# rounak-meyur/revs-admm

Hardware: NVIDIA B200
Metric: home_hours_scheduled_per_sec (higher is better)
Workload: dtype f64

## Files before the change

revs-admm_b200/csrc/kernels.cuh:

```cuda
#pragma once
#include <vector>

#include "common.cuh"

namespace revs {

struct HomeParams {
    const double* load;
    const double* p_est;
    const double* p_sch;
    const int* iter;
    const double* gamma;
    const double* cost;
    const uint8_t* has_ev;
    const double* rating;
    const int* start;
    const int* end;
    const int* n_min;
    const int* n_max;
    double* p_sch_new;
    double* p_ev;
    double* dsum;
    int first;
    int* infeasible;
// ... 47 lines not shown
    ResidualOut* res;
    PeerReduce peer;
    double* partials;
    int Hp, T;
    double kappa, tol, count;
};

cudaError_t launch_dual_update(const DualParams& P, cudaStream_t stream);

struct QpParams {
    const FeederDev* feeders;
    const double* Rpool;
    const double* rn2;
    const double* rmax;
    int* cand;
    int* queue;
    const double* z_t;
    double* lam_t;
    double* g_t;
    double* v_t;
    void* gbf_t;
    const float* v32_t;
    int* wcount;
    int* widx;
    int* status;
    int* inner_ok;
    int* n_running;
    unsigned long long* newton_its;
    int* max_ws;
    unsigned long long* flops;
    unsigned long long* cols;
    int* n_failed;
    int* cls;
    int* n_cls;
    const int* order;
    const int* order_count;
    int4* order4;
    int sweep;
    int list0, nlists;
    int list_extra;
    int warp_m_max;
    int warp_m_max_big;
    int ncols;
    long long* trace;
    unsigned long long* dbg;
    int T;
    int64_t Hp;
    double u, tol;
    int init;
    int inner_max;
    int* round_ctr;
    unsigned long long cond_round;
    int use_cond;
};

struct RoundEndParams {
    const int* n_running;
    const int* n_failed;
    const int* infeasible;
    int* round_ctr;
    int* noconv;
    unsigned long long* rounds_total;
    int round_max;
    unsigned long long cond_round;
    int use_cond;
};
cudaError_t launch_round_end(const RoundEndParams& P, cudaStream_t stream);

struct ClassGateParams {
    const int* order_count;
    unsigned long long cond[kQpClasses];
    int first_gated;
};
cudaError_t launch_class_gate(const ClassGateParams& P, cudaStream_t stream);
cudaError_t qp_warp_prepare();
cudaError_t screen_prepare();
cudaError_t screen_tc5_prepare();

cudaError_t launch_utility_qp(const QpParams& P, int grid, int cls, cudaStream_t stream);
int qp_warp_max_n();
cudaError_t launch_qp_init(const QpParams& P, int max_warp_n, cudaStream_t stream);
int qp_warp_ctas_per_sm();
int qp_warp_m_max_default();
cudaError_t launch_utility_qp_warp(const QpParams& P, int nj, int ctas_per_sm, cudaStream_t stream);
cudaError_t launch_utility_qp_fast(const QpParams& P, cudaStream_t stream);
cudaError_t launch_order_columns(const QpParams& P, int mode, int* order, int* order_count, cudaStream_t stream);

struct NewtonZone {
    int feeder;
    int nn, nlev, n;
    int wn;
    int col0;
    int64_t node_off;
    int64_t home_off;
    int64_t lvl_off;
    int64_t ws_off;
    double scale;
};
struct NewtonParams {
    const NewtonZone* zones;
    int n_zones;
    const int* lvl;
    const int* parent;
    const int2* child;
    const int2* homes;
    const double* rho;
    const int* hlist;
    const int* hnode;
    double* ws;
    double4* ws4;
    double2* ws2;
    int* wsi;
    int64_t ws_stride;
    const FeederDev* feeders;
    const double* z_t;
    double* lam_t;
    double* g_t;
    int* status;
    int* inner_ok;
    int* wcount;
    int* noconv;
    double* dbg_dump;
    int dbg_dump_col, dbg_dump_outer, dbg_dump_guess;
    double* dbg_trace;
    int* dbg_col;
    unsigned long long* newton_its;
    unsigned long long* cols;
    unsigned long long* flops;
    int* max_ws;
    int T;
    int64_t Hp;
    double u, tol;
};
struct NewtonZoneHost {
    std::vector<int> lvl, parent, child0, nchild, home0, nhome, hlist, hnode;
    std::vector<double> rho;
    double scale = 1.0;
};
void newton_build_zone(int n_nodes, const int* parent, const double* r, int n_res, const int* res_node, NewtonZoneHost& Z);
cudaError_t launch_tree_newton(const NewtonParams& P, int n_cols, cudaStream_t stream);
constexpr int kNewtonWsDoubles = 18, kNewtonWs4 = 3, kNewtonWs2 = 2, kNewtonWsInts = 3;

int contract_tile_rows(int T);
cudaError_t launch_contract(const ContractProblem* d_problems, const ContractTile* d_tiles, int n_tiles,
                            int T, int mode, double v2, cudaStream_t stream);

cudaError_t launch_gather_wait(const unsigned long long* flags, int world, unsigned long long seq, int* timeout, cudaStream_t s);

int screen_tile_rows();
cudaError_t launch_to_bf16(const double* in, void* out, size_t n, cudaStream_t s);
cudaError_t launch_screen(const ScreenProblem* d_problems, const ContractTile* d_tiles, int n_tiles, int T, double thr,
                          cudaStream_t stream);

int screen_tc5_tile_rows();
size_t screen_tc5_map_bytes();
uint32_t screen_tc5_box_rows_a();
uint32_t screen_tc5_box_rows_b();
cudaError_t screen_tc5_encode(void* host_map, const void* gptr, uint64_t rows, uint64_t cols, uint64_t pitch_elems,
                              uint32_t box_rows);
cudaError_t launch_screen_tc5(const ScreenProblem* d_problems, const ContractTile* d_tiles, int n_tiles, const void* d_maps_a,
                              const void* d_map_b, const int* d_b_col0, int T, double thr, cudaStream_t stream);

cudaError_t launch_sens_voltage(const int* parent, const double* cumr, const int* row_node,
                                const int* res_node, int n_rows, int n_res, double* out, int ld,
                                cudaStream_t s);
cudaError_t launch_sens_voltage_batched(const FeederDev* feeders, int n_feeders, int max_n, const int64_t* node_off,
// ... 171 lines not shown
```

revs-admm_b200/csrc/revs_capi.cu:

```cuda
#include <chrono>
#include <cstdarg>
#include <cstdio>
#include <cstring>
#include <algorithm>
#include <cstdlib>
#include <cmath>
#include <mutex>
#include <string>
#include <vector>

#include "../../include/revs_admm.h"
#include "kernels.cuh"

using namespace revs;

namespace {

thread_local std::string g_err;

int fail(int code, const char* fmt, ...) {
    char buf[512];
    va_list ap;
    va_start(ap, fmt);
    vsnprintf(buf, sizeof buf, fmt, ap);
// ... 962 lines not shown
    const size_t HT = (size_t)hp * T;

#define TRY(x)                                                                                     \
    do {                                                                                           \
        cudaError_t e_ = (x);                                                                      \
        if (e_ != cudaSuccess) {                                                                   \
            free_all(s);                                                                           \
            delete s;                                                                              \
            return fail(REVS_ERR_CUDA, "%s failed: %s", #x, cudaGetErrorString(e_));               \
        }                                                                                          \
    } while (0)
    int prio_lo = 0, prio_hi = 0;
    TRY(cudaDeviceGetStreamPriorityRange(&prio_lo, &prio_hi));
    s->prio_lo = prio_lo;
    s->prio_hi = prio_hi;
    TRY(cudaStreamCreateWithPriority(&s->sU, cudaStreamNonBlocking, prio_hi));
    TRY(cudaStreamCreateWithPriority(&s->sH, cudaStreamNonBlocking, prio_lo));
    TRY(cudaEventCreateWithFlags(&s->evV, cudaEventDisableTiming));
    for (int cl = 0; cl < kQpClasses; ++cl) {
        TRY(cudaStreamCreateWithPriority(&s->sQ[cl], cudaStreamNonBlocking, prio_hi));
        TRY(cudaEventCreateWithFlags(&s->evQ[cl], cudaEventDisableTiming));
    }
    TRY(cudaEventCreateWithFlags(&s->evHomeDone, cudaEventDisableTiming));
    TRY(cudaEventCreateWithFlags(&s->evDualDone, cudaEventDisableTiming));
    TRY(cudaEventCreate(&s->evT0));
    TRY(cudaEventCreate(&s->evT1));
    TRY(dalloc(&s->d_feeders, (size_t)n_feeders));
    TRY(cudaMemcpy(s->d_feeders, s->feeders.data(), sizeof(FeederDev) * n_feeders, cudaMemcpyHostToDevice));
    TRY(dalloc(&s->d_Rpool, (size_t)rp));
    TRY(dalloc(&s->d_rn2, (size_t)hp));
    TRY(dalloc(&s->d_rmax, (size_t)hp));
    TRY(dalloc(&s->d_cand, (size_t)s->ncols));
    TRY(dalloc(&s->d_stage, (size_t)s->H * (T + 1)));
    {
        std::vector<int64_t> hmap((size_t)s->H);
        for (int f = 0; f < n_feeders; ++f)
            for (int64_t i = feeder_off[f]; i < feeder_off[f + 1]; ++i) hmap[i] = s->feeders[f].off + (i - feeder_off[f]);
        TRY(dalloc(&s->d_hmap, hmap.size()));
        TRY(cudaMemcpy(s->d_hmap, hmap.data(), hmap.size() * sizeof(int64_t), cudaMemcpyHostToDevice));
    }
    s->Rpool_elems = (size_t)rp;
    TRY(cudaMalloc(&s->d_Rbf, (size_t)(rp ? rp : 1) * 2));
    TRY(cudaMemset(s->d_Rbf, 0, (size_t)(rp ? rp : 1) * 2));
    TRY(cudaMalloc(&s->d_gbf, HT * 2));
    TRY(cudaMemset(s->d_gbf, 0, HT * 2));
    TRY(dalloc(&s->d_v32, HT));
    if (getenv("REVS_EXACT_GEMM")) s->screen = false;
    TRY(dalloc(&s->d_load, HT));
    TRY(dalloc(&s->d_pest, HT));
    TRY(dalloc(&s->d_psch[0], HT));
    TRY(dalloc(&s->d_psch[1], HT));
    TRY(dalloc(&s->d_gamma, HT));
    TRY(dalloc(&s->d_pev, HT));
    TRY(dalloc(&s->d_soc, (size_t)hp * (T + 1)));
    TRY(dalloc(&s->d_has_ev, (size_t)hp));
    TRY(dalloc(&s->d_rating, (size_t)hp));
    TRY(dalloc(&s->d_capacity, (size_t)hp));
    TRY(dalloc(&s->d_initial, (size_t)hp));
    TRY(dalloc(&s->d_indconst, (size_t)hp));
    TRY(dalloc(&s->d_start, (size_t)hp));
    TRY(dalloc(&s->d_end, (size_t)hp));
    TRY(dalloc(&s->d_nmin, (size_t)hp));
    TRY(dalloc(&s->d_nmax, (size_t)hp));
    TRY(dalloc(&s->d_zero_i, (size_t)hp));
    TRY(dalloc(&s->d_cost, (size_t)T));
    TRY(dalloc(&s->d_zt, HT));
    TRY(dalloc(&s->d_lamt, HT));
    TRY(dalloc(&s->d_gt, HT));
    TRY(dalloc(&s->d_vt, HT));
    TRY(dalloc(&s->d_wcount, (size_t)s->ncols));
    TRY(dalloc(&s->d_widx, (size_t)s->ncols * kWMax));
    TRY(dalloc(&s->d_status, (size_t)s->ncols));
    TRY(dalloc(&s->d_innerok, (size_t)s->ncols));
    TRY(dalloc(&s->d_cls, (size_t)s->ncols));
    TRY(dalloc(&s->d_order, (size_t)s->ncols * kQpClasses));
    TRY(dalloc(&s->d_order4, (size_t)s->ncols * (kQpLists - kQpClasses)));
    if (hp >= (int64_t)1 << 31 || (rp >> 4) >= (int64_t)1 << 31) s->use_warp_kernel = false;
    TRY(dalloc(&s->d_order_count, (size_t)2 * kQpLists));
    TRY(dalloc(&s->d_cnt, (size_t)1));
    TRY(dalloc(&s->d_respart, (size_t)2 * ((hp + 31) / 32)));
    TRY(dalloc(&s->d_dsum, (size_t)hp));
    {
        const char* e;
        s->warp_m_max = (e = getenv("REVS_WARP_M_MAX")) ? atoi(e) : qp_warp_m_max_default();
        s->warp_m_max_big = (e = getenv("REVS_WARP_M_MAX_BIG")) ? atoi(e) : s->warp_m_max;
        s->use_fast = !((e = getenv("REVS_NO_FAST")) && atoi(e));
        s->debug = getenv("REVS_DEBUG") != nullptr;
        s->debug_host = getenv("REVS_DEBUG_HOST") != nullptr;
        if ((e = getenv("REVS_NO_GRAPH")) && atoi(e)) s->use_graph = false;
        if ((e = getenv("REVS_DEBUG_TRACE")) && sscanf(e, "%d,%d", &s->trace_iter, &s->trace_round) == 2) s->use_graph = false;
        if ((e = getenv("REVS_DEBUG_TRACE_FILE"))) s->trace_file = e;
        if (s->debug) s->use_graph = false;
    }
    TRY(cudaHostAlloc((void**)&s->h_cnt, sizeof(Counters), cudaHostAllocDefault));
    memset(s->h_cnt, 0, sizeof(Counters));

    {
        int rc2 = build_tables(s);
        if (rc2) { free_all(s); delete s; return rc2; }
    }
#undef TRY
    *out = s;
    return REVS_OK;
}

int revs_destroy(revs_solver* s) {
    if (!s) return REVS_OK;
    free_all(s);
    delete s;
    return REVS_OK;
}

int revs_set_sensitivity(revs_solver* s, int feeder, const double* R_res) {
    if (!s || !R_res || feeder < 0 || feeder >= s->nf) return fail(REVS_ERR_ARG, "bad arguments");
    CU(cudaSetDevice(s->device));
    const FeederDev& fd = s->feeders[feeder];
    if (s->roff_alloc[feeder] < 0)
        return fail(REVS_ERR_ARG, "feeder %d has %d residences (> %d): it runs on its tree, give it with "
                    "revs_set_feeder_tree(s) instead of a dense block", feeder, fd.n, kDenseMaxN);
    if (s->is_newton[feeder]) {
        int rc = set_newton(s, feeder, false);
        if (rc) return rc;
        s->nt_host[feeder] = NewtonZoneHost();
        if ((rc = build_tables(s)) || (rc = rebuild_newton(s))) return rc;
    }
    for (int64_t i = 0; i < (int64_t)fd.n * fd.n; ++i)
        if (!(R_res[i] >= 0.0)) return fail(REVS_ERR_ARG, "sensitivity block of feeder %d has a negative or NaN entry", feeder);
    if (fd.n)
        CU(cudaMemcpy2D(s->d_Rpool + fd.roff, (size_t)fd.np * sizeof(double), R_res, (size_t)fd.n * sizeof(double),
                        (size_t)fd.n * sizeof(double), fd.n, cudaMemcpyHostToDevice));
    s->sens_set[feeder] = 1;
    s->rn2_valid = false;
    return REVS_OK;
}

int revs_set_feeder_tree(revs_solver* s, int feeder, int n_nodes, const int32_t* parent, const double* r,
                         const int32_t* res_node) {
    if (!s || !parent || !r || !res_node || feeder < 0 || feeder >= s->nf || n_nodes <= 0)
        return fail(REVS_ERR_ARG, "bad arguments");
    CU(cudaSetDevice(s->device));
    const FeederDev& fd = s->feeders[feeder];
    std::vector<double> cumr(n_nodes);
    for (int i = 0; i < n_nodes; ++i) {
        if (parent[i] >= i || parent[i] < -1) return fail(REVS_ERR_ARG, "nodes must be topologically ordered (parent[i] < i)");
        if (!(r[i] >= 0.0)) return fail(REVS_ERR_ARG, "negative or NaN resistance at node %d", i);
        cumr[i] = (parent[i] < 0 ? 0.0 : cumr[parent[i]]) + r[i];
    }
    for (int j = 0; j < fd.n; ++j)
        if (res_node[j] < 0 || res_node[j] >= n_nodes) return fail(REVS_ERR_ARG, "res_node[%d] out of range", j);
    Tree& t = s->trees[feeder];
    if (t.d_parent && !t.pooled) { cudaFree(t.d_parent); cudaFree(t.d_cumr); cudaFree(t.d_res_node); }
    t = Tree();
    s->net.valid = false;
    s->net.central_valid = false;
    t.n_nodes = n_nodes;
    CU(dalloc(&t.d_parent, (size_t)n_nodes));
    CU(dalloc(&t.d_cumr, (size_t)n_nodes));
    CU(dalloc(&t.d_res_node, (size_t)fd.np));
    CU(cudaMemcpy(t.d_parent, parent, sizeof(int) * n_nodes, cudaMemcpyHostToDevice));
    CU(cudaMemcpy(t.d_cumr, cumr.data(), sizeof(double) * n_nodes, cudaMemcpyHostToDevice));
    CU(cudaMemcpy(t.d_res_node, res_node, sizeof(int) * fd.n, cudaMemcpyHostToDevice));
    {
        const bool want = fd.n > s->newton_min_n || s->roff_alloc[feeder] < 0;
        if (want != (bool)s->is_newton[feeder]) {
            int rc = set_newton(s, feeder, want);
            if (rc || (rc = build_tables(s))) return rc;
        }
    }
// ... 1454 lines not shown
```

revs-admm_b200/csrc/utility_qp_warp.cu:

```cuda
#include <cstdlib>

#include <cuda_bf16.h>

#include "kernels.cuh"

namespace revs {

namespace {

#ifndef REVS_WARPS_PER_CTA
#define REVS_WARPS_PER_CTA 4
#endif
constexpr int kWarpsPerCta = REVS_WARPS_PER_CTA;
constexpr int kCtasPerSm = 16 / kWarpsPerCta;
constexpr int kHW = kWW + 1;
constexpr int kCacheDoubles = 1024;
constexpr double kArcMinW = 9.5367431640625e-07;
constexpr int kPdasMaxW = 40;
constexpr double kHessShiftW = 1e-12;
constexpr int kAddMaxW = 8;
constexpr int kPassMaxW = 10;
constexpr int kRecheckMaxW = 256;
constexpr int kHysteresisW = 8;

template <int CACHE>
struct WarpSmemT {
    double H[kWW * kHW];
    double L[kWW * kHW];
    double rows[CACHE];
};
#ifndef REVS_WARP_CTAS_SMALL
#define REVS_WARP_CTAS_SMALL (8 / REVS_WARPS_PER_CTA)
#endif
#ifndef REVS_WARP_CTAS_BIG
#define REVS_WARP_CTAS_BIG (8 / REVS_WARPS_PER_CTA)
#endif
#ifndef REVS_WARP_CACHE_BIG
#define REVS_WARP_CACHE_BIG 2560
#endif
template <int NJ> struct WarpCfg {
    static constexpr int kCache = NJ <= 4 ? kCacheDoubles : REVS_WARP_CACHE_BIG;
    static constexpr int kCtas = NJ <= 8 ? (NJ <= 4 ? kCtasPerSm : REVS_WARP_CTAS_SMALL) : REVS_WARP_CTAS_BIG;
};

struct WarpStats {
    unsigned long long its = 0;
    double flops = 0.0;
    int handed = 0, deferred = 0, max_ws = 0, cols = 0;
};

__device__ __forceinline__ double warp_bcast(double v, int src) { return __shfl_sync(0xffffffffu, v, src); }

template <int NJ>
__device__ __forceinline__ void recheck_rows(unsigned candk, const double* __restrict__ R, int ld, int n,
                                             const double (&gj)[NJ], double (&vub)[NJ]) {
    const int lane = threadIdx.x & 31;
    const unsigned full = 0xffffffffu;
    if (!__any_sync(full, candk != 0u)) return;
#pragma unroll 1
    for (int k = 0; k < NJ; ++k) {
        unsigned cand = __ballot_sync(full, (candk >> k) & 1u);
        while (cand) {
            int s[4], cnt = 0;
#pragma unroll
            for (int q = 0; q < 4; ++q) {
                if (cand) { s[q] = __ffs(cand) - 1; cand &= cand - 1; ++cnt; }
                else s[q] = s[0];
            }
            double a[4] = {0.0, 0.0, 0.0, 0.0};
#pragma unroll
            for (int kk = 0; kk < NJ; ++kk) {
                const int jj = lane + 32 * kk;
                if (jj < n) {
#pragma unroll
                    for (int q = 0; q < 4; ++q) a[q] = fma(R[(size_t)(s[q] + 32 * k) * ld + jj], gj[kk], a[q]);
                }
            }
#pragma unroll
            for (int o = 16; o > 0; o >>= 1) {
#pragma unroll
                for (int q = 0; q < 4; ++q) a[q] += __shfl_xor_sync(full, a[q], o);
            }
            double mine = 0.0;
            bool hit = false;
#pragma unroll
            for (int q = 0; q < 4; ++q)
                if (q < cnt && lane == s[q]) { mine = a[q]; hit = true; }
            if (hit) {
#pragma unroll
                for (int kk = 0; kk < NJ; ++kk)
                    if (kk == k) vub[kk] = mine;
            }
        }
    }
}

template <int NJ>
__device__ __forceinline__ void solve_column(const QpParams& P, const int4 ent, WarpSmemT<WarpCfg<NJ>::kCache>& sm, WarpStats& st) {
    constexpr int kCacheD = WarpCfg<NJ>::kCache;
    const int lane = threadIdx.x & 31;
    const unsigned full = 0xffffffffu;
    const int c = ent.x;
    const int n = ent.z & 0xffff, ld = ent.z >> 16;
    const int t = c % P.T;
    const size_t hoff = (size_t)ent.y;
    const double* __restrict__ R = P.Rpool + ((size_t)ent.w << 4);
    const size_t col = (size_t)t * P.Hp + hoff;
    const double* z = P.z_t + col;
    double* lam_g = P.lam_t + col;
    double* g = P.g_t + col;
    const double u = P.u, tol = P.tol;
    int* widx = P.widx + (size_t)c * kWMax;
    const int m_old = P.wcount[c];
    const bool solved_before = P.inner_ok[c] == 1;
    const int wi = lane < kWW ? widx[lane] : 0;

    long long tr_start = 0;
    if (P.trace) asm volatile("mov.u64 %0, %%globaltimer;" : "=l"(tr_start));
    const long long tr_clk0 = clock64();
    const double thr = (1.0 - kScreenMargin) * u;

    double zj[NJ], gj[NJ], g0[NJ], vub[NJ];
    unsigned inw = 0;
    unsigned candk = 0;
    if (P.v32_t) {
        const float* v32 = P.v32_t + col;
        float vf[NJ];
#pragma unroll
        for (int k = 0; k < NJ; ++k) {
            const int jc = min(lane + 32 * k, n - 1);
            zj[k] = z[jc];
            gj[k] = g[jc];
            vf[k] = v32[jc];
        }
        if (lane < (n + 15) / 16) asm volatile("prefetch.global.L2 [%0];" ::"l"(P.rmax + hoff + 16 * lane));
#pragma unroll
        for (int k = 0; k < NJ; ++k) {
            const bool in = lane + 32 * k < n;
            if (!in) { zj[k] = 0.0; gj[k] = 0.0; }
            g0[k] = gj[k];
            const double a = in ? (double)vf[k] : 0.0;
            vub[k] = kScreenUp * a;
            if (in && a > thr) candk |= 1u << k;
        }
    } else {
        const double* v64 = P.v_t + col;
#pragma unroll
        for (int k = 0; k < NJ; ++k) {
            const int jc = min(lane + 32 * k, n - 1);
            zj[k] = z[jc];
            gj[k] = g[jc];
            vub[k] = v64[jc];
        }
#pragma unroll
        for (int k = 0; k < NJ; ++k) {
            if (lane + 32 * k >= n) { zj[k] = 0.0; gj[k] = 0.0; vub[k] = 0.0; }
            g0[k] = gj[k];
        }
    }

    int idx = 0, m = 0;
    double lam = 0.0;
    if (m_old > 0) {
        const double l = lane < m_old ? lam_g[wi] : 0.0;
        const unsigned keep = __ballot_sync(full, lane < m_old && l > 0.0);
        m = __popc(keep);
        const int src = __fns(keep, 0, lane + 1);
        const int si = __shfl_sync(full, wi, src & 31);
        const double sl = __shfl_sync(full, l, src & 31);
        if (lane < m) { idx = si; lam = sl; }
#pragma unroll 1
        for (int a = 0; a < m; ++a) {
            const int h = __shfl_sync(full, idx, a);
            if ((h & 31) == lane) inw |= 1u << (h >> 5);
        }
        candk &= ~inw;
    }

    double flops = 0.0;
    int its_total = 0;
    bool changed = false;
    long long tph[4] = {0, 0, 0, 0}, tq0 = clock64(), tq1;
    int npass = 0;
#define WPHASE(i) do { if (P.trace) { tq1 = clock64(); tph[i] += tq1 - tq0; tq0 = tq1; } } while (0)
    auto trace_out = [&](int kind) {
        if (P.trace && lane == 0) {
            long long tr_end; unsigned smid;
            asm volatile("mov.u64 %0, %%globaltimer;" : "=l"(tr_end));
            asm volatile("mov.u32 %0, %%smid;" : "=r"(smid));
            long long* rec = P.trace + 12 * (size_t)c;
            rec[0] = tr_start; rec[1] = tr_end; rec[2] = smid; rec[3] = ((long long)m << 20) | its_total;
            for (int i = 0; i < 4; ++i) rec[4 + i] = tph[i];
            rec[8] = npass; rec[9] = kind; rec[10] = m_old; rec[11] = clock64() - tr_clk0;
        }
    };
    tph[0] = tq0 - tr_clk0;
    int exit_kind = 0, reason = 0;
    double grad = 0.0;

    for (int pass = 0;; ++pass) {
        recheck_rows<NJ>(candk, R, ld, n, gj, vub);
        candk = 0;
        WPHASE(pass == 0 ? 0 : 3);

        if (pass > 0) {
            const bool row = lane < m;
            unsigned drop = __ballot_sync(full, row && !(lam > 0.0));
            if (drop) {
                const unsigned keep = __ballot_sync(full, row && lam > 0.0);
                while (drop) {
                    const int a = __ffs(drop) - 1;
                    drop &= drop - 1;
                    const int h = __shfl_sync(full, idx, a);
                    const double vr = u - warp_bcast(grad, a);
                    if ((h & 31) == lane) {
#pragma unroll
                        for (int k = 0; k < NJ; ++k)
                            if (k == (h >> 5)) { vub[k] = vr; inw &= ~(1u << k); }
                    }
                }
                m = __popc(keep);
                const int src = __fns(keep, 0, lane + 1);
                const int si = __shfl_sync(full, idx, src & 31);
                const double sl = __shfl_sync(full, lam, src & 31);
                idx = lane < m ? si : 0;
                lam = lane < m ? sl : 0.0;
            }
        }

        int added = 0;
        bool left = false;
        const int room = min(kAddMaxW, kWW - m);
#pragma unroll 1
        for (int r = 0; r <= room; ++r) {
            double best = -1.0;
            int bj = 0x7fffffff;
#pragma unroll
            for (int k = 0; k < NJ; ++k) {
                const int j = lane + 32 * k;
                const double viol = vub[k] - u;
                if (j < n && !((inw >> k) & 1u) && viol > tol && viol > best) { best = viol; bj = j; }
            }
            if (!__any_sync(full, best >= 0.0)) break;
#pragma unroll
            for (int o = 16; o > 0; o >>= 1) {
                const double ob = __shfl_xor_sync(full, best, o);
                const int oj = __shfl_xor_sync(full, bj, o);
                if (ob > best || (ob == best && oj < bj)) { best = ob; bj = oj; }
            }
            if (r == room) { left = true; break; }
            if (lane == m + added) { idx = bj; lam = 0.0; }
            if ((bj & 31) == lane) inw |= 1u << (bj >> 5);
            ++added;
        }
        if (added == 0 && !left) {
            if (pass > 0 || m == 0 || solved_before) break;
        }
        if ((left && m + added == kWW) || pass >= kPassMaxW) { exit_kind = 2; reason = pass >= kPassMaxW ? 2 : 1; break; }
        m += added;
        ++npass;
        const bool row = lane < m;

        const int ncache = min(m, kCacheD / ld);
        __syncwarp();
        {
            const int nchunk = (n + 1) >> 1;
#pragma unroll 1
            for (int a = 0; a < ncache; ++a) {
                const double* src = R + (size_t)__shfl_sync(full, idx, a) * ld;
                const unsigned dst = (unsigned)__cvta_generic_to_shared(sm.rows + a * ld);
                for (int ch = lane; ch < nchunk; ch += 32)
                    asm volatile("cp.async.cg.shared.global [%0], [%1], 16;" ::"r"(dst + 16u * ch), "l"(src + 2 * ch) : "memory");
            }
            asm volatile("cp.async.commit_group;" ::: "memory");
            asm volatile("cp.async.wait_group 0;" ::: "memory");
        }
        __syncwarp();
        auto rowp = [&](int a) -> const double* {
            const int ia = __shfl_sync(full, idx, a);
            return a < ncache ? sm.rows + a * ld : R + (size_t)ia * ld;
        };

        int ok = 0, its = 0;
        bool bail = false;
        WPHASE(1);

        if (m == 1) {
            const double* rp = rowp(0);
            double r1[NJ];
#pragma unroll
            for (int k = 0; k < NJ; ++k) {
                const int j = lane + 32 * k;
                r1[k] = j < n ? rp[j] : 0.0;
            }
            const double l_in = warp_bcast(lam, 0);
            double l = l_in;
#pragma unroll 1
            for (int it = 0; it < 48; ++it) {
                double v = 0.0, S = 0.0;
#pragma unroll
                for (int k = 0; k < NJ; ++k) {
                    const double gk = fmax(zj[k] - r1[k] * l, 0.0);
                    gj[k] = gk;
                    v = fma(r1[k], gk, v);
                    if (gk > 0.0) S = fma(r1[k], r1[k], S);
                }
#pragma unroll
                for (int o = 16; o > 0; o >>= 1) {
                    v += __shfl_xor_sync(full, v, o);
                    S += __shfl_xor_sync(full, S, o);
                }
                ++its;
                const double fr = v - u;
                if ((l > 0.0 ? fabs(fr) : fmax(fr, 0.0)) < tol) { ok = 1; grad = -fr; break; }
                double ln = S > 0.0 ? l + fr / S : 0.0;
                if (ln < 0.0) ln = 0.0;
                if (ln == l) break;
                l = ln;
            }
            flops += 4.0 * n * its;
            lam = lane == 0 ? l : 0.0;
            if (l != l_in) changed = true;
            if (ok && l == l_in) its = 0;
            if (!ok) its = 0;
        }

        if (!ok) {
            const double scale = warp_sum(row ? P.rn2[hoff + idx] : 0.0) / (double)max(m, 1);
            const double shift = kHessShiftW * scale + 1e-300;
            double phi;
            {
                double acc = 0.0;
#pragma unroll
                for (int k = 0; k < NJ; ++k) acc = fma(gj[k], gj[k], acc);
                phi = 0.5 * warp_sum(acc) + u * warp_sum(row ? lam : 0.0);
            }
            double hrow[kWW];
#pragma unroll
            for (int q = 0; q < kWW; ++q) hrow[q] = 0.0;
            unsigned fbits = 0;
            bool have_H = false;
// ... 19 lines not shown
                if (kkt < tol) { ok = 1; break; }

                {
                    int nupd = 0;
                    unsigned nowmask = 0;
#pragma unroll
                    for (int k = 0; k < NJ; ++k)
                        if (gj[k] > 0.0) nowmask |= 1u << k;
                    if (!have_H) {
#pragma unroll 1
                        for (int p = 0; p < m; ++p) {
                            const double* rp_ptr = rowp(p);
                            double rp[NJ];
#pragma unroll
                            for (int k = 0; k < NJ; ++k) {
                                const int j = lane + 32 * k;
                                rp[k] = (j < n && gj[k] > 0.0) ? rp_ptr[j] : 0.0;
                            }
#pragma unroll 1
                            for (int q = 0; q <= p; q += 2) {
                                const double* r0 = rowp(q);
                                const double* r1 = rowp(min(q + 1, p));
                                double a0 = 0.0, a1 = 0.0;
#pragma unroll
                                for (int k = 0; k < NJ; ++k) {
                                    const int j = lane + 32 * k;
                                    if (j < n) { a0 = fma(rp[k], r0[j], a0); a1 = fma(rp[k], r1[j], a1); }
                                }
#pragma unroll
                                for (int o = 16; o > 0; o >>= 1) {
                                    a0 += __shfl_xor_sync(full, a0, o);
                                    a1 += __shfl_xor_sync(full, a1, o);
                                }
                                if (lane == p) {
#pragma unroll
                                    for (int qq = 0; qq < kWW; ++qq) {
                                        if (qq == q) hrow[qq] = a0;
                                        if (qq == q + 1 && q + 1 <= p) hrow[qq] = a1;
                                    }
                                }
                            }
                        }
                        nupd = __reduce_add_sync(full, __popc(nowmask));
                    } else {
#pragma unroll 1
                        for (int k = 0; k < NJ; ++k) {
                            const bool now = (nowmask >> k) & 1u;
                            const bool was = (fbits >> k) & 1u;
                            unsigned chg = __ballot_sync(full, now != was);
                            const unsigned nowb = __ballot_sync(full, now);
                            while (chg) {
                                const int src = __ffs(chg) - 1;
                                chg &= chg - 1;
                                const int j = src + 32 * k;
                                const double sgn = ((nowb >> src) & 1u) ? 1.0 : -1.0;
                                const double ra = row ? (lane < ncache ? sm.rows[lane * ld + j] : R[(size_t)idx * ld + j]) : 0.0;
#pragma unroll
                                for (int q = 0; q < kWW; ++q) {
                                    const double rq = warp_bcast(ra, q);
                                    if (q <= lane) hrow[q] = fma(sgn * ra, rq, hrow[q]);
                                }
                                ++nupd;
                            }
                        }
                    }
                    fbits = nowmask;
                    have_H = true;
                    flops += (double)m * (m + 1) * nupd;
                    __syncwarp();
#pragma unroll
                    for (int q = 0; q < kWW; ++q)
                        if (row && q <= lane) { sm.H[lane * kHW + q] = hrow[q]; sm.H[q * kHW + lane] = hrow[q]; }
                    __syncwarp();
                }

                double b = 0.0;
#pragma unroll 1
                for (int q = 0; q < m; ++q) {
                    const double lq = warp_bcast(lam, q);
                    if (row && lq != 0.0) b = fma(sm.H[lane * kHW + q], lq, b);
                }
                b += shift * lam - grad;
                bool inA = row && (lam > 0.0 || grad < 0.0);
                double x = 0.0;
                bool pdas_ok = false;
#pragma unroll 1
                for (int guess = 0; guess < kPdasMaxW; ++guess) {
                    const unsigned Am = __ballot_sync(full, inA);
                    const int ma = __popc(Am);
                    const int pos = __popc(Am & ((1u << lane) - 1));
                    double xs = 0.0;
                    if (ma > 0) {
                        const int o = (lane < ma) ? (int)__fns(Am, 0, lane + 1) : 0;
#pragma unroll 1
                        for (int cidx = 0; cidx < ma; ++cidx) {
                            const int oc = __shfl_sync(full, o, cidx);
                            if (lane < ma && cidx <= lane) sm.L[lane * kHW + cidx] = sm.H[o * kHW + oc] + (cidx == lane ? shift : 0.0);
                        }
                        __syncwarp();
                        double rdiag = 1.0;
#pragma unroll 1
                        for (int k2 = 0; k2 < ma; ++k2) {
                            double sv = 0.0;
                            if (lane >= k2 && lane < ma) {
                                sv = sm.L[lane * kHW + k2];
                                for (int p2 = 0; p2 < k2; ++p2) sv = fma(-sm.L[lane * kHW + p2], sm.L[k2 * kHW + p2], sv);
                            }
                            const double skk = fmax(warp_bcast(sv, k2), 1e-300);
                            const double rk = rsqrt(skk);
                            const double dkk = skk * rk;
                            if (lane == k2) rdiag = rk;
                            if (lane >= k2 && lane < ma) sm.L[lane * kHW + k2] = lane == k2 ? dkk : sv * rk;
                            __syncwarp();
                        }
                        double y = warp_bcast(b, o);
                        if (lane >= ma) y = 0.0;
#pragma unroll 1
                        for (int k2 = 0; k2 < ma; ++k2) {
                            const double yk = warp_bcast(y, k2) * warp_bcast(rdiag, k2);
                            if (lane == k2) y = yk;
                            if (lane > k2 && lane < ma) y = fma(-sm.L[lane * kHW + k2], yk, y);
                        }
#pragma unroll 1
                        for (int k2 = ma - 1; k2 >= 0; --k2) {
                            const double xk = warp_bcast(y, k2) * warp_bcast(rdiag, k2);
                            if (lane == k2) y = xk;
                            if (lane < k2) y = fma(-sm.L[k2 * kHW + lane], xk, y);
                        }
                        xs = y;
                        flops += (2.0 / 3.0) * ma * ma * ma + 4.0 * ma * ma + 2.0 * m * ma;
                    }
                    const double xg = warp_bcast(xs, pos & 31);
                    x = inA ? xg : 0.0;
                    double mu = 0.0;
#pragma unroll 1
                    for (int q = 0; q < m; ++q) {
                        const double xq = warp_bcast(x, q);
                        if (row && xq != 0.0) mu = fma(sm.H[lane * kHW + q], xq, mu);
                    }
                    mu -= b;
                    const bool bad = row && (inA ? (x <= 0.0) : (mu < 0.0));
                    if (!__any_sync(full, bad)) { pdas_ok = true; break; }
                    if (bad) inA = !inA;
                }
                if (!pdas_ok) { bail = true; reason = 3; break; }

                const double dir = x - lam;
                double gt[NJ];
                double alpha = 1.0, phin = phi, lt = lam;
                bool stepped = false;
#pragma unroll 1
                for (; alpha >= kArcMinW; alpha *= 0.5) {
                    lt = row ? fmax(fma(alpha, dir, lam), 0.0) : 0.0;
                    {
                        double pi[NJ];
#pragma unroll
                        for (int k = 0; k < NJ; ++k) pi[k] = 0.0;
#pragma unroll 1
                        for (int a = 0; a < m; ++a) {
                            const double la = warp_bcast(lt, a);
                            const double* rr = rowp(a);
                            if (la != 0.0) {
#pragma unroll
                                for (int k = 0; k < NJ; ++k) {
                                    const int j = lane + 32 * k;
                                    if (j < n) pi[k] = fma(rr[j], la, pi[k]);
                                }
                            }
                        }
                        double acc = 0.0;
#pragma unroll
                        for (int k = 0; k < NJ; ++k) {
                            const int j = lane + 32 * k;
                            gt[k] = j < n ? fmax(zj[k] - pi[k], 0.0) : 0.0;
                            acc = fma(gt[k], gt[k], acc);
                        }
                        phin = 0.5 * warp_sum(acc) + u * warp_sum(row ? lt : 0.0);
                    }
                    flops += 2.0 * m * n;
                    const double slope = warp_sum(row ? grad * (lt - lam) : 0.0);
                    if (phin <= phi + 1e-4 * slope + 1e-14 * fabs(phi)) { stepped = true; break; }
                }
                if (!stepped) { bail = true; reason = 4; break; }
                lam = lt;
                phi = phin;
                changed = true;
#pragma unroll
                for (int k = 0; k < NJ; ++k) gj[k] = gt[k];
            }
        }
        its_total += its;
        WPHASE(2);
        if (bail || !ok) { exit_kind = 2; if (!reason) reason = 5; break; }

        double dp = 0.0;
#pragma unroll
        for (int k = 0; k < NJ; ++k) dp += fmax(gj[k] - g0[k], 0.0);
        dp = warp_sum(dp) * (1.0 + 1e-9);
        int ncand = 0;
        {
            const double* rmax = P.rmax + hoff;
            double rm[NJ];
#pragma unroll
            for (int k = 0; k < NJ; ++k) rm[k] = rmax[min(lane + 32 * k, n - 1)];
#pragma unroll
            for (int k = 0; k < NJ; ++k) {
                const int j = lane + 32 * k;
                if (j < n && !((inw >> k) & 1u)) {
                    const double bnd = dp > 0.0 ? fma(rm[k], dp, vub[k]) : vub[k];
                    if (bnd - u > tol) { candk |= 1u << k; ++ncand; }
                    else vub[k] = bnd;
                }
            }
            ncand = __reduce_add_sync(full, ncand);
        }
#pragma unroll
        for (int k = 0; k < NJ; ++k) g0[k] = gj[k];
        flops += 2.0 * n * min(ncand, kRecheckMaxW);
        if (ncand == 0) break;
        if (ncand > kRecheckMaxW) { exit_kind = 1; break; }
    }
    WPHASE(3);

    if (exit_kind == 2) {
        if (lane == 0) { P.cls[c] = 1; P.inner_ok[c] = 2; }
        ++st.handed;
        trace_out(2 + 16 * reason);
        return;
    }
    if (changed || m != m_old) {
        if (lane < m_old) lam_g[wi] = 0.0;
        __syncwarp();
        if (lane < m) { lam_g[idx] = lam; widx[lane] = idx; }
        if (changed) {
            __nv_bfloat16* gbf = P.gbf_t ? reinterpret_cast<__nv_bfloat16*>(P.gbf_t) + col : nullptr;
#pragma unroll
            for (int k = 0; k < NJ; ++k) {
                const int j = lane + 32 * k;
                if (j < n) {
                    g[j] = gj[k];
                    if (gbf) gbf[j] = __float2bfloat16_rn((float)gj[k]);
                }
            }
        }
    }
    if (lane == 0) {
        P.wcount[c] = m;
        P.inner_ok[c] = 1;
        if (exit_kind == 0) P.status[c] = 1;
    }
    if (exit_kind == 1) ++st.deferred;
    trace_out(exit_kind);
    st.its += (unsigned long long)its_total;
    st.flops += flops;
    st.max_ws = max(st.max_ws, m);
#undef WPHASE
}

}

__global__ void __launch_bounds__(256) qp_init_kernel(QpParams P, int max_warp_n) {
    const int lane = threadIdx.x & 31;
    const int c = blockIdx.x * (blockDim.x >> 5) + (threadIdx.x >> 5);
    if (blockIdx.x == 0 && threadIdx.x == 0 && P.round_ctr) {
        *P.round_ctr = 0;
        if (P.use_cond) cudaGraphSetConditional((cudaGraphConditionalHandle)P.cond_round, 1u);
    }
    if (c >= P.ncols) return;
    const int f = c / P.T, t = c % P.T;
    const FeederDev fd = P.feeders[f];
    const int n = fd.n, ld = fd.np;
    if (fd.roff < 0) {
        if (lane == 0) { P.cls[c] = 0; P.status[c] = 1; P.inner_ok[c] = 1; if (P.cand) P.cand[c] = 0; }
        return;
    }
    const double* R = P.Rpool + fd.roff;
    const size_t col = (size_t)t * P.Hp + fd.off;
    const double* z = P.z_t + col;
    double* lam_g = P.lam_t + col;
    double* g = P.g_t + col;
    __nv_bfloat16* gbf = P.gbf_t ? reinterpret_cast<__nv_bfloat16*>(P.gbf_t) + col : nullptr;
    int* widx = P.widx + (size_t)c * kWMax;

    int m = 0;
    if (P.init == 2) {
        const int wc = P.wcount[c];
        if (wc == 0) {
            if (lane == 0) {
                P.cls[c] = n <= max_warp_n ? 0 : 1;
                P.status[c] = 0;
                P.inner_ok[c] = 0;
                if (P.cand) P.cand[c] = 0;
            }
            return;
        }
        for (int a0 = 0; a0 < wc; a0 += 32) {
            const int a = a0 + lane;
            const int i = a < wc ? widx[a] : 0;
            const bool on = a < wc && lam_g[i] > 0.0;
            const unsigned bal = __ballot_sync(0xffffffffu, on);
            __syncwarp();
            if (on) widx[m + __popc(bal & ((1u << lane) - 1))] = i;
            m += __popc(bal);
        }
    } else {
        for (int j0 = 0; j0 < n; j0 += 32) {
            const int j = j0 + lane;
            const bool on = j < n && lam_g[j] > 0.0;
            const unsigned bal = __ballot_sync(0xffffffffu, on);
            if (on) {
                const int pos = m + __popc(bal & ((1u << lane) - 1));
                if (pos < kWMax) widx[pos] = j;
                else lam_g[j] = 0.0;
            }
            m += __popc(bal);
        }
        m = min(m, kWMax);
    }
    __syncwarp();
    int cl = (n <= max_warp_n && m <= (n <= 128 ? P.warp_m_max : P.warp_m_max_big)) ? 0 : 1;
    while (cl < kQpClasses - 1 && m > qp_class_cap(cl)) ++cl;

    for (int j0 = 0; j0 < n; j0 += 32) {
        const int j = j0 + lane;
        if (j >= n) break;
        double pi = 0.0;
        for (int a = 0; a < m; ++a) {
            const int i = widx[a];
            pi = fma(R[(size_t)i * ld + j], lam_g[i], pi);
        }
        const double gj = fmax(z[j] - pi, 0.0);
        g[j] = gj;
        if (gbf) gbf[j] = __float2bfloat16_rn((float)gj);
    }
    if (lane == 0) {
// ... 240 lines not shown
                    if (gbf) gbf[j] = __float2bfloat16_rn((float)gj[k]);
                }
            }
            its_sum += (unsigned long long)its;
        }
        maxws = max(maxws, m_new);
        __syncwarp();
    }
    if (lane == 0) {
        if (its_sum) atomicAdd(P.newton_its, its_sum);
        if (flops > 0.0) atomicAdd(P.flops, (unsigned long long)flops);
        if (maxws) atomicMax(P.max_ws, maxws);
        if (cols - passed > 0) atomicAdd(P.cols, (unsigned long long)(cols - passed));
        if (P.dbg && passed) atomicAdd(P.dbg + 3, (unsigned long long)passed);
    }
}

cudaError_t launch_utility_qp_fast(const QpParams& P, cudaStream_t stream) {
    int dev = 0, n_sm = 0;
    cudaError_t e = cudaGetDevice(&dev);
    if (e == cudaSuccess) e = cudaDeviceGetAttribute(&n_sm, cudaDevAttrMultiProcessorCount, dev);
    if (e != cudaSuccess) return e;
    utility_qp_fast_kernel<<<n_sm * 4, 32 * kFastWarps, 0, stream>>>(P);
    return cudaGetLastError();
}

int qp_warp_max_n() { return kWarpMaxN; }

static int g_warp_n_sm[4][64] = {};

template <int NJ>
static cudaError_t prepare_warp_nj(int* n_sm_out) {
    const int smem = (int)sizeof(WarpSmemT<WarpCfg<NJ>::kCache>) * kWarpsPerCta;
    int* n_sm = g_warp_n_sm[(NJ - 4) / 2];
    int dev = 0;
    cudaError_t e = cudaGetDevice(&dev);
    if (e != cudaSuccess) return e;
    dev &= 63;
    if (!n_sm[dev]) {
        int n = 0;
        e = cudaDeviceGetAttribute(&n, cudaDevAttrMultiProcessorCount, dev);
        if (e == cudaSuccess) e = cudaFuncSetAttribute(utility_qp_warp_kernel<NJ>, cudaFuncAttributeMaxDynamicSharedMemorySize, smem);
#ifndef REVS_WARP_NO_CARVEOUT
        if (e == cudaSuccess) e = cudaFuncSetAttribute(utility_qp_warp_kernel<NJ>, cudaFuncAttributePreferredSharedMemoryCarveout, cudaSharedmemCarveoutMaxShared);
#endif
        if (e != cudaSuccess) return e;
        n_sm[dev] = n;
    }
    if (n_sm_out) *n_sm_out = n_sm[dev];
    return cudaSuccess;
}

cudaError_t qp_warp_prepare() {
    cudaError_t e = prepare_warp_nj<4>(nullptr);
    if (e == cudaSuccess) e = prepare_warp_nj<6>(nullptr);
    if (e == cudaSuccess) e = prepare_warp_nj<8>(nullptr);
    if (e == cudaSuccess) e = prepare_warp_nj<10>(nullptr);
    return e;
}

template <int NJ>
static cudaError_t launch_warp_nj(const QpParams& P, int ctas_per_sm, cudaStream_t stream) {
    const int smem = (int)sizeof(WarpSmemT<WarpCfg<NJ>::kCache>) * kWarpsPerCta;
    int nsm = 0;
    cudaError_t e = prepare_warp_nj<NJ>(&nsm);
    if (e != cudaSuccess) return e;
    int n_sm[1] = {nsm};
    const int dev = 0;
    const int cmax = WarpCfg<NJ>::kCtas;
    ctas_per_sm = ctas_per_sm < 1 ? 1 : (ctas_per_sm > cmax ? cmax : ctas_per_sm);
    utility_qp_warp_kernel<NJ><<<n_sm[dev] * ctas_per_sm, 32 * kWarpsPerCta, smem, stream>>>(P);
    return cudaGetLastError();
}

cudaError_t launch_utility_qp_warp(const QpParams& P, int nj, int ctas_per_sm, cudaStream_t stream) {
    if (nj == 10) return launch_warp_nj<10>(P, ctas_per_sm, stream);
    if (nj == 8) return launch_warp_nj<8>(P, ctas_per_sm, stream);
    if (nj == 6) return launch_warp_nj<6>(P, ctas_per_sm, stream);
    return launch_warp_nj<4>(P, ctas_per_sm, stream);
}

int qp_warp_ctas_per_sm() { return kCtasPerSm; }
int qp_warp_m_max_default() { return kWW - kHysteresisW; }

}
```

Before: 267.5 million.

## Add safeguarded PDAS fallback in warp QP and defer columns instead of bailing

```diff
diff --git a/profiles/exp_warp_finish.py b/profiles/exp_warp_finish.py
--- /dev/null
+++ b/profiles/exp_warp_finish.py
@@ -0,0 +1,132 @@
+import json
+import os
+import re
+import sys
+import tempfile
+
+import numpy as np
+
+ROOT = os.path.dirname(os.path.dirname(os.path.abspath(__file__)))
+sys.path.insert(0, ROOT)
+import bench
+import revs_admm_b200 as R
+
+REASONS = {1: "full set", 2: "passes", 3: "pdas", 4: "line search", 5: "other"}
+
+
+def solve_once(prob, env, graph):
+    trees, hm, cost, sizes, T = prob
+    old = {k: os.environ.get(k) for k in env}
+    os.environ.update(env)
+    fd, path = tempfile.mkstemp(suffix=".log")
+    saved = os.dup(2)
+    os.dup2(fd, 2)
+    try:
+        with R.Solver(sizes, T) as s:
+            s.set_option("graph", 1 if graph else 0)
+            s.set_feeder_trees(trees)
+            s.set_homes(**hm)
+            s.set_tariff(cost)
+            s.solve_admm(**bench.ADMM)
+            st = s.stats()
+    finally:
+        os.dup2(saved, 2)
+        os.close(saved)
+        os.close(fd)
+        for k, v in old.items():
+            if v is None:
+                os.environ.pop(k, None)
+            else:
+                os.environ[k] = v
+    with open(path) as f:
+        log = f.read()
+    os.unlink(path)
+    return st, log
+
+
+def rounds_by_iteration(log):
+    pat = re.compile(r"admm (\d+) round (\d+): running (\d+) by class (\d+)/(\d+)/(\d+)/(\d+)")
+    out = {}
+    for m in pat.finditer(log):
+        k, r, run, c0, c1, c2, c3 = map(int, m.groups())
+        out.setdefault(k, []).append({"round": r, "running_after": run, "by_class": [c0, c1, c2, c3]})
+    return out
+
+
+def read_trace(path):
+    return np.fromfile(path, dtype=np.int64).reshape(-1, 12)
+
+
+def main():
+    wl = sys.argv[1] if len(sys.argv) > 1 else "synthetic-refshape-125k-homes-per-gpu-x96"
+    out_path = sys.argv[2] if len(sys.argv) > 2 else None
+    prob = bench.make_rank_problem(wl, 0)
+    sizes = prob[3]
+    res = {"workload": wl, "lib": os.environ.get("REVS_LIB", "default"), "zones": len(sizes),
+           "zone_size": [int(min(sizes)), int(max(sizes))]}
+
+    st, log = solve_once(prob, {"REVS_DEBUG": "1"}, graph=False)
+    rb = rounds_by_iteration(log)
+    res["host_loop"] = {"admm_iterations": st["admm_iterations"], "qp_outer_iterations": st["qp_outer_iterations"],
+                        "max_working_set": st["max_working_set"], "qp_ms": st["qp_ms"], "total_ms": st["total_ms"],
+                        "rounds_per_iteration": {k: len(v) for k, v in sorted(rb.items())},
+                        "class1_after_round0": {k: v[0]["by_class"][1] for k, v in sorted(rb.items())}}
+    tails = [k for k, v in sorted(rb.items()) if len(v) > 1]
+    print(f"host-driven: {st['admm_iterations']} iterations, {st['qp_outer_iterations']} working-set rounds, "
+          f"max |W| {st['max_working_set']}; iterations with a tail round: {tails}")
+
+    traces = []
+    tmpdir = tempfile.mkdtemp()
+    for k in tails[:3]:
+        rec = {"iteration": k}
+        for r in (0, 1):
+            path = os.path.join(tmpdir, f"tr_{k}_{r}.bin")
+            solve_once(prob, {"REVS_DEBUG_TRACE": f"{k},{r}", "REVS_DEBUG_TRACE_FILE": path}, graph=False)
+            rec[f"round{r}"] = read_trace(path)
+        t0, t1 = rec["round0"], rec["round1"]
+        ran0 = t0[:, 1] > 0
+        is_cta0 = (t0[:, 3] >> 40) > 0
+        warp0 = ran0 & ~is_cta0
+        kind0 = t0[:, 9] & 15
+        handed = np.nonzero(warp0 & (kind0 == 2))[0]
+        cta0 = np.nonzero(ran0 & is_cta0)[0]
+        item = {"iteration": k,
+                "round0": {"warp_columns": int(warp0.sum()), "class1_columns": int(cta0.size),
+                           "handed": [{"column": int(c), "reason": REASONS.get(int(t0[c, 9] >> 4), "?"),
+                                       "m": int((t0[c, 3] >> 20) & 0xFFFFF), "m_stored": int(t0[c, 10]),
+                                       "passes": int(t0[c, 8]), "pieces": int(t0[c, 3] & 0xFFFFF)} for c in handed]}}
+        ran1 = np.nonzero(t1[:, 1] > 0)[0]
+        cols1 = []
+        for c in ran1:
+            cols1.append({"column": int(c), "class": int(t1[c, 3] >> 40),
+                          "origin": "handed by the warp kernel" if c in set(handed.tolist())
+                          else ("class 1 in round 0" if c in set(cta0.tolist()) else "other"),
+                          "m": int((t1[c, 3] >> 20) & 0xFFFFF), "pieces": int(t1[c, 3] & 0xFFFFF),
+                          "pdas_guesses": int(t1[c, 9]), "phi_evals": int(t1[c, 10]),
+                          "us": float((t1[c, 1] - t1[c, 0]) * 1e-3)})
+        item["round1"] = cols1
+        traces.append(item)
+        print(f"iteration {k}: round 0 handed {len(handed)} ({[h['reason'] for h in item['round0']['handed']]}), "
+              f"class-1 columns in round 0: {cta0.size}; round 1 columns: {[(c['origin'], c['m'], c['us']) for c in cols1]}")
+    res["traces"] = traces
+
+    s = R.PipelinedSolver(sizes, prob[4], pipelines=4)
+    try:
+        s.set_feeder_trees(prob[0])
+        s.set_homes(**prob[1])
+        s.set_tariff(prob[2])
+        s.solve_admm(**bench.ADMM)
+        per = [p.stats() for p in s.parts]
+    finally:
+        s.close()
+    res["pipelines4"] = [{"admm_iterations": p["admm_iterations"], "qp_outer_iterations": p["qp_outer_iterations"],
+                          "max_working_set": p["max_working_set"]} for p in per]
+    print("4 pipelines, captured loop: rounds per pipeline", [p["qp_outer_iterations"] for p in per],
+          "ADMM iterations", [p["admm_iterations"] for p in per])
+    if out_path:
+        with open(out_path, "w") as f:
+            json.dump(res, f, indent=1)
+
+
+if __name__ == "__main__":
+    main()
diff --git a/revs-admm_b200/csrc/kernels.cuh b/revs-admm_b200/csrc/kernels.cuh
--- a/revs-admm_b200/csrc/kernels.cuh
+++ b/revs-admm_b200/csrc/kernels.cuh
@@ -153,6 +153,7 @@
 cudaError_t launch_qp_init(const QpParams& P, int max_warp_n, cudaStream_t stream);
 int qp_warp_ctas_per_sm();
 int qp_warp_m_max_default();
+int qp_warp_m_max_big_default();
 cudaError_t launch_utility_qp_warp(const QpParams& P, int nj, int ctas_per_sm, cudaStream_t stream);
 cudaError_t launch_utility_qp_fast(const QpParams& P, cudaStream_t stream);
 cudaError_t launch_order_columns(const QpParams& P, int mode, int* order, int* order_count, cudaStream_t stream);
diff --git a/revs-admm_b200/csrc/revs_capi.cu b/revs-admm_b200/csrc/revs_capi.cu
--- a/revs-admm_b200/csrc/revs_capi.cu
+++ b/revs-admm_b200/csrc/revs_capi.cu
@@ -1068,8 +1068,9 @@
     TRY(dalloc(&s->d_dsum, (size_t)hp));
     {
         const char* e;
-        s->warp_m_max = (e = getenv("REVS_WARP_M_MAX")) ? atoi(e) : qp_warp_m_max_default();
-        s->warp_m_max_big = (e = getenv("REVS_WARP_M_MAX_BIG")) ? atoi(e) : s->warp_m_max;
+        const char* e_all = getenv("REVS_WARP_M_MAX");
+        s->warp_m_max = e_all ? atoi(e_all) : qp_warp_m_max_default();
+        s->warp_m_max_big = (e = getenv("REVS_WARP_M_MAX_BIG")) ? atoi(e) : (e_all ? s->warp_m_max : qp_warp_m_max_big_default());
         s->use_fast = !((e = getenv("REVS_NO_FAST")) && atoi(e));
         s->debug = getenv("REVS_DEBUG") != nullptr;
         s->debug_host = getenv("REVS_DEBUG_HOST") != nullptr;
diff --git a/revs-admm_b200/csrc/utility_qp_warp.cu b/revs-admm_b200/csrc/utility_qp_warp.cu
--- a/revs-admm_b200/csrc/utility_qp_warp.cu
+++ b/revs-admm_b200/csrc/utility_qp_warp.cu
@@ -19,7 +19,7 @@
 constexpr int kPdasMaxW = 40;
 constexpr double kHessShiftW = 1e-12;
 constexpr int kAddMaxW = 8;
-constexpr int kPassMaxW = 10;
+constexpr int kPassMaxW = 16;
 constexpr int kRecheckMaxW = 256;
 constexpr int kHysteresisW = 8;
 
@@ -98,6 +98,7 @@
 template <int NJ>
 __device__ __forceinline__ void solve_column(const QpParams& P, const int4 ent, WarpSmemT<WarpCfg<NJ>::kCache>& sm, WarpStats& st) {
     constexpr int kCacheD = WarpCfg<NJ>::kCache;
+    constexpr bool kSafeguard = NJ > 4;
     const int lane = threadIdx.x & 31;
     const unsigned full = 0xffffffffu;
     const int c = ent.x;
@@ -196,7 +197,9 @@
     };
     tph[0] = tq0 - tr_clk0;
     int exit_kind = 0, reason = 0;
+    bool solved = true;
     double grad = 0.0;
+    double tau = 1.0;
 
     for (int pass = 0;; ++pass) {
         recheck_rows<NJ>(candk, R, ld, n, gj, vub);
@@ -256,7 +259,8 @@
         if (added == 0 && !left) {
             if (pass > 0 || m == 0 || solved_before) break;
         }
-        if ((left && m + added == kWW) || pass >= kPassMaxW) { exit_kind = 2; reason = pass >= kPassMaxW ? 2 : 1; break; }
+        if (left && added == 0 && pass > 0) { exit_kind = 2; reason = 1; break; }
+        if (pass >= kPassMaxW) { exit_kind = 1; reason = 2; break; }
         m += added;
         ++npass;
         const bool row = lane < m;
@@ -442,11 +446,16 @@
                 }
                 b += shift * lam - grad;
                 bool inA = row && (lam > 0.0 || grad < 0.0);
-                double x = 0.0;
-                bool pdas_ok = false;
-#pragma unroll 1
-                for (int guess = 0; guess < kPdasMaxW; ++guess) {
-                    const unsigned Am = __ballot_sync(full, inA);
+                const bool fre = row && !(lam <= fmin(1e-8, kkt) && grad > 0.0);
+                bool safe = false;
+                double gt[NJ];
+                double alpha = 1.0, phin = phi, lt = lam;
+                bool stepped = false;
+#pragma unroll 1
+                for (int guess = 0;;) {
+                    const bool inS = safe ? fre : inA;
+                    const double shs = safe ? 1e-10 * tau * scale + 1e-300 : shift;
+                    const unsigned Am = __ballot_sync(full, inS);
                     const int ma = __popc(Am);
                     const int pos = __popc(Am & ((1u << lane) - 1));
                     double xs = 0.0;
@@ -455,7 +464,7 @@
 #pragma unroll 1
                         for (int cidx = 0; cidx < ma; ++cidx) {
                             const int oc = __shfl_sync(full, o, cidx);
-                            if (lane < ma && cidx <= lane) sm.L[lane * kHW + cidx] = sm.H[o * kHW + oc] + (cidx == lane ? shift : 0.0);
+                            if (lane < ma && cidx <= lane) sm.L[lane * kHW + cidx] = sm.H[o * kHW + oc] + (cidx == lane ? shs : 0.0);
                         }
                         __syncwarp();
                         double rdiag = 1.0;
@@ -473,7 +482,7 @@
                             if (lane >= k2 && lane < ma) sm.L[lane * kHW + k2] = lane == k2 ? dkk : sv * rk;
                             __syncwarp();
                         }
-                        double y = warp_bcast(b, o);
+                        double y = warp_bcast(safe ? -grad : b, o);
                         if (lane >= ma) y = 0.0;
 #pragma unroll 1
                         for (int k2 = 0; k2 < ma; ++k2) {
@@ -491,57 +500,68 @@
                         flops += (2.0 / 3.0) * ma * ma * ma + 4.0 * ma * ma + 2.0 * m * ma;
                     }
                     const double xg = warp_bcast(xs, pos & 31);
-                    x = inA ? xg : 0.0;
-                    double mu = 0.0;
-#pragma unroll 1
-                    for (int q = 0; q < m; ++q) {
-                        const double xq = warp_bcast(x, q);
-                        if (row && xq != 0.0) mu = fma(sm.H[lane * kHW + q], xq, mu);
+                    const double x = inS ? xg : 0.0;
+                    if (!safe) {
+                        ++guess;
+                        double mu = 0.0;
+#pragma unroll 1
+                        for (int q = 0; q < m; ++q) {
+                            const double xq = warp_bcast(x, q);
+                            if (row && xq != 0.0) mu = fma(sm.H[lane * kHW + q], xq, mu);
+                        }
+                        mu -= b;
+                        const bool bad = row && (inA ? (x <= 0.0) : (mu < 0.0));
+                        if (__any_sync(full, bad)) {
+                            if (bad) inA = !inA;
+                            if (guess >= kPdasMaxW) {
+                                if (!kSafeguard) { bail = true; reason = 3; break; }
+                                safe = true;
+                            }
+                            continue;
+                        }
                     }
-                    mu -= b;
-                    const bool bad = row && (inA ? (x <= 0.0) : (mu < 0.0));
-                    if (!__any_sync(full, bad)) { pdas_ok = true; break; }
-                    if (bad) inA = !inA;
-                }
-                if (!pdas_ok) { bail = true; reason = 3; break; }
-
-                const double dir = x - lam;
-                double gt[NJ];
-                double alpha = 1.0, phin = phi, lt = lam;
-                bool stepped = false;
-#pragma unroll 1
-                for (; alpha >= kArcMinW; alpha *= 0.5) {
-                    lt = row ? fmax(fma(alpha, dir, lam), 0.0) : 0.0;
-                    {
-                        double pi[NJ];
-#pragma unroll
-                        for (int k = 0; k < NJ; ++k) pi[k] = 0.0;
-#pragma unroll 1
-                        for (int a = 0; a < m; ++a) {
-                            const double la = warp_bcast(lt, a);
-                            const double* rr = rowp(a);
-                            if (la != 0.0) {
-#pragma unroll
-                                for (int k = 0; k < NJ; ++k) {
-                                    const int j = lane + 32 * k;
-                                    if (j < n) pi[k] = fma(rr[j], la, pi[k]);
+
+                    const double dir = safe ? (inS ? x : -lam) : x - lam;
+#pragma unroll 1
+                    for (alpha = 1.0; alpha >= kArcMinW; alpha *= 0.5) {
+                        lt = row ? fmax(fma(alpha, dir, lam), 0.0) : 0.0;
+                        {
+                            double pi[NJ];
+#pragma unroll
+                            for (int k = 0; k < NJ; ++k) pi[k] = 0.0;
+#pragma unroll 1
+                            for (int a = 0; a < m; ++a) {
+                                const double la = warp_bcast(lt, a);
+                                const double* rr = rowp(a);
+                                if (la != 0.0) {
+#pragma unroll
+                                    for (int k = 0; k < NJ; ++k) {
+                                        const int j = lane + 32 * k;
+                                        if (j < n) pi[k] = fma(rr[j], la, pi[k]);
+                                    }
                                 }
                             }
+                            double acc = 0.0;
+#pragma unroll
+                            for (int k = 0; k < NJ; ++k) {
+                                const int j = lane + 32 * k;
+                                gt[k] = j < n ? fmax(zj[k] - pi[k], 0.0) : 0.0;
+                                acc = fma(gt[k], gt[k], acc);
+                            }
+                            phin = 0.5 * warp_sum(acc) + u * warp_sum(row ? lt : 0.0);
                         }
-                        double acc = 0.0;
-#pragma unroll
-                        for (int k = 0; k < NJ; ++k) {
-                            const int j = lane + 32 * k;
-                            gt[k] = j < n ? fmax(zj[k] - pi[k], 0.0) : 0.0;
-                            acc = fma(gt[k], gt[k], acc);
-                        }
-                        phin = 0.5 * warp_sum(acc) + u * warp_sum(row ? lt : 0.0);
+                        flops += 2.0 * m * n;
+                        const double slope = warp_sum(row ? grad * (lt - lam) : 0.0);
+                        if (phin <= phi + 1e-4 * slope + 1e-14 * fabs(phi)) { stepped = true; break; }
                     }
-                    flops += 2.0 * m * n;
-                    const double slope = warp_sum(row ? grad * (lt - lam) : 0.0);
-                    if (phin <= phi + 1e-4 * slope + 1e-14 * fabs(phi)) { stepped = true; break; }
-                }
-                if (!stepped) { bail = true; reason = 4; break; }
+                    if (stepped) break;
+                    if (!kSafeguard) { bail = true; reason = 4; break; }
+                    if (!safe) { safe = true; continue; }
+                    if (tau > 1e40 || ma == 0) break;
+                    tau *= 1e3;
+                }
+                if (bail) break;
+                if (safe && alpha == 1.0) tau = fmax(1.0, tau / 10.0);
                 lam = lt;
                 phi = phin;
                 changed = true;
@@ -551,7 +571,8 @@
         }
         its_total += its;
         WPHASE(2);
-        if (bail || !ok) { exit_kind = 2; if (!reason) reason = 5; break; }
+        if (bail) { exit_kind = 2; break; }
+        if (!ok) { exit_kind = 1; reason = 5; solved = false; break; }
 
         double dp = 0.0;
 #pragma unroll
@@ -606,11 +627,11 @@
     }
     if (lane == 0) {
         P.wcount[c] = m;
-        P.inner_ok[c] = 1;
+        P.inner_ok[c] = solved ? 1 : 0;
         if (exit_kind == 0) P.status[c] = 1;
     }
     if (exit_kind == 1) ++st.deferred;
-    trace_out(exit_kind);
+    trace_out(exit_kind + 16 * reason);
     st.its += (unsigned long long)its_total;
     st.flops += flops;
     st.max_ws = max(st.max_ws, m);
@@ -1017,5 +1038,6 @@
 
 int qp_warp_ctas_per_sm() { return kCtasPerSm; }
 int qp_warp_m_max_default() { return kWW - kHysteresisW; }
-
-}
+int qp_warp_m_max_big_default() { return kWW; }
+
+}
```

After: 279.5 million, median of 6. +4.5%, better.
